# Thitrongdan202/Digital-Watermarking-for-image-Video-using-DCT-SVD-Singular-Value-Decomposition

Measured on AMD Instinct MI355X. Metric: frames/sec embed+extract @4K Y-channel, higher is better.
Workload: dtype f32

## Files before the change

### digital-watermarking-for-image-video-using-dct-svd-singular-value-decomposition_amd/csrc/wmhip.hip

```cpp
#include <hip/hip_runtime.h>
#include <stdio.h>
#include <stdlib.h>
#include <string.h>
#include <new>

#include "wm_internal.h"
#include "wm_tile_math.h"

using namespace wmi;

namespace wmi {

thread_local char g_err[512] = "";

int set_err(int code, const char* fmt, const char* a, const char* b) {
  snprintf(g_err, sizeof(g_err), fmt, a, b);
  return code;
}

int grow(wm_ctx* ctx, void** buf, size_t* have, size_t bytes, const char* what) {
  if (bytes <= *have) return WM_OK;
  if (*buf) {
    WM_HIP(hipStreamSynchronize(ctx->stream));
    WM_HIP(hipFree(*buf));
    *buf = nullptr; *have = 0;
  }
  const size_t mb = (size_t)1 << 20;
  const size_t want = (bytes + mb - 1) / mb * mb;
  if (hipMalloc(buf, want) != hipSuccess) {
    (void)hipGetLastError();
    *buf = nullptr;
    return set_err(WM_ERR_NOMEM, "hipMalloc failed for %s", what);
  }
  *have = want;
  return WM_OK;
}

}

namespace {

constexpr int N_SUMS = 5;

#if !defined(WM_NO_ASM_JACOBI)
#include "wm_jacobi_gfx950.inc"
#if !__has_include("wm_jacobi_sigma_gfx950.inc")
#error "wm_jacobi_sigma_gfx950.inc is generated: run `python tools/gen_jacobi_asm.py --write` (build() does) before compiling"
#endif
#include "wm_jacobi_sigma_gfx950.inc"
#endif

__device__ __forceinline__ int sigma_tile_dev(const wm::RawTile& raw, float (&s)[8]) {
#if !defined(WM_NO_ASM_JACOBI)
  float n2[8];
  constexpr float SIGMA_SKIP2 = 1e-8f;
  constexpr int SIGMA_SKIP_FROM = 2;
  const unsigned long long more = jacobi_sigma_gfx950(raw.lo, raw.hi, n2, wm::JAC_CONV2_SIGMA, SIGMA_SKIP2, 3, SIGMA_SKIP_FROM);
#pragma unroll
  for (int i = 0; i < 8; ++i) s[i] = wm::fsqrt(n2[i]);
  return more ? -1 : 1;
#else
  return wm::sigma_tile_pk(raw, s);
#endif
}

template <bool ALIGNED>
__device__ __forceinline__ uint32_t load_px4(const uint8_t* __restrict__ q) {
  if (ALIGNED) return *reinterpret_cast<const uint32_t*>(q);
  return q[0] | (q[1] << 8) | (q[2] << 16) | ((uint32_t)q[3] << 24);
}
template <bool ALIGNED>
__device__ __forceinline__ void store_px4(uint8_t* __restrict__ q, const uint32_t w) {
  if (ALIGNED) { *reinterpret_cast<uint32_t*>(q) = w; return; }
#pragma unroll
  for (int i = 0; i < 4; ++i) q[i] = (uint8_t)(w >> (8 * i));
}
template <bool ALIGNED>
__device__ __forceinline__ void load_px8(const uint8_t* __restrict__ q, uint32_t& lo, uint32_t& hi) {
  if (ALIGNED) { const uint2 w = *reinterpret_cast<const uint2*>(q); lo = w.x; hi = w.y; }
  else { lo = load_px4<false>(q); hi = load_px4<false>(q + 4); }
}
template <bool ALIGNED>
__device__ __forceinline__ void store_px8(uint8_t* __restrict__ q, const uint32_t lo, const uint32_t hi) {
  if (ALIGNED) *reinterpret_cast<uint2*>(q) = make_uint2(lo, hi);
  else { store_px4<false>(q, lo); store_px4<false>(q + 4, hi); }
}

template <bool ALIGNED>
__device__ __forceinline__ void load_raw(const uint8_t* __restrict__ p, const size_t stride, wm::RawTile& t) {
#pragma unroll
  for (int r = 0; r < 8; ++r) load_px8<ALIGNED>(p + r * stride, t.lo[r], t.hi[r]);
}

template <bool ALIGNED>
__device__ __forceinline__ void load_tile_u8(const uint8_t* __restrict__ p, const size_t stride, float (&a)[8][8]) {
#pragma unroll
  for (int r = 0; r < 8; ++r) {
    uint32_t lo, hi;
    load_px8<ALIGNED>(p + r * stride, lo, hi);
    a[r][0] = (float)(lo & 0xffu); a[r][1] = (float)((lo >> 8) & 0xffu);
    a[r][2] = (float)((lo >> 16) & 0xffu); a[r][3] = (float)(lo >> 24);
    a[r][4] = (float)(hi & 0xffu); a[r][5] = (float)((hi >> 8) & 0xffu);
    a[r][6] = (float)((hi >> 16) & 0xffu); a[r][7] = (float)(hi >> 24);
  }
}

template <bool ALIGNED>
__device__ __forceinline__ void store_tile_u8(uint8_t* __restrict__ p, const size_t stride, const float (&a)[8][8]) {
#pragma unroll
  for (int r = 0; r < 8; ++r) {
    const uint32_t lo = wm::quant_u8(a[r][0]) | (wm::quant_u8(a[r][1]) << 8) |
                        (wm::quant_u8(a[r][2]) << 16) | (wm::quant_u8(a[r][3]) << 24);
    const uint32_t hi = wm::quant_u8(a[r][4]) | (wm::quant_u8(a[r][5]) << 8) |
                        (wm::quant_u8(a[r][6]) << 16) | (wm::quant_u8(a[r][7]) << 24);
    store_px8<ALIGNED>(p + r * stride, lo, hi);
  }
}

template <bool ALIGNED>
__device__ __forceinline__ void load_words(const uint8_t* __restrict__ p, const size_t stride, uint32_t (&w)[8]) {
#pragma unroll
  for (int r = 0; r < 8; ++r) w[r] = load_px4<ALIGNED>(p + r * stride);
}
template <bool ALIGNED>
__device__ __forceinline__ void store_words(uint8_t* __restrict__ p, const size_t stride, const uint32_t (&w)[8]) {
#pragma unroll
  for (int r = 0; r < 8; ++r) store_px4<ALIGNED>(p + r * stride, w[r]);
}

template <bool VEC>
__device__ __forceinline__ void load_row8_f32(const float* __restrict__ p, float (&row)[8]) {
  if (VEC) {
    const float4 x = *reinterpret_cast<const float4*>(p);
    const float4 y = *reinterpret_cast<const float4*>(p + 4);
    row[0] = x.x; row[1] = x.y; row[2] = x.z; row[3] = x.w;
    row[4] = y.x; row[5] = y.y; row[6] = y.z; row[7] = y.w;
  } else {
#pragma unroll
    for (int i = 0; i < 8; ++i) row[i] = p[i];
  }
}

template <bool VEC>
__device__ __forceinline__ void store_row8_f32(float* __restrict__ p, const float (&row)[8]) {
  if (VEC) {
    *reinterpret_cast<float4*>(p) = make_float4(row[0], row[1], row[2], row[3]);
    *reinterpret_cast<float4*>(p + 4) = make_float4(row[4], row[5], row[6], row[7]);
  } else {
#pragma unroll
    for (int i = 0; i < 8; ++i) p[i] = row[i];
  }
}

__device__ __forceinline__ void load_mat_f32(const float* __restrict__ p, float (&m)[8][8]) {
#pragma unroll
  for (int r = 0; r < 8; ++r) load_row8_f32<true>(p + r * 8, m[r]);
}
__device__ __forceinline__ void store_mat_f32(float* __restrict__ p, const float (&m)[8][8]) {
#pragma unroll
  for (int r = 0; r < 8; ++r) store_row8_f32<true>(p + r * 8, m[r]);
}

struct Geom {
  int nbx;
  int n_tiles;
  int W;
  size_t HW;
  size_t row_stride;
  size_t plane_stride;
};

#define STRIDED_TILE(base, g, plane, ty, tx) \
  ((base) + (plane) * (g).plane_stride + (size_t)(ty) * 8 * (g).row_stride + (size_t)(tx) * 8)
#define DENSE_TILE(out, g, plane, ty, tx) ((out) + (plane) * (g).HW + (size_t)(ty) * 8 * (g).W + (size_t)(tx) * 8)

__device__ __forceinline__ bool tile_coords(const Geom& g, int& t, int& ty, int& tx) {
  t = blockIdx.x * WAVE + threadIdx.x;
  if (t >= g.n_tiles) return false;
  ty = t / g.nbx;
  tx = t - ty * g.nbx;
  return true;
}

constexpr unsigned N_XCD = 8;
struct GroupPlane { unsigned grp; size_t plane; };
__device__ __forceinline__ GroupPlane group_plane_planefast(const unsigned n_planes) {
  const unsigned b = blockIdx.x, x = b % N_XCD, k = b / N_XCD;
  return {x + N_XCD * (k / n_planes), k % n_planes};
}
__device__ __forceinline__ bool tile_coords_planefast(const Geom& g, const unsigned n_planes, int& t, int& ty,
                                                      int& tx, size_t& plane) {
  const GroupPlane gp = group_plane_planefast(n_planes);
  plane = gp.plane;
  t = (int)(gp.grp * WAVE + threadIdx.x);
  if (t >= g.n_tiles) return false;
  ty = t / g.nbx;
  tx = t - ty * g.nbx;
  return true;
}
inline dim3 tile_grid_planefast(const Geom& g, int n_planes) {
  const size_t groups = ((size_t)g.n_tiles + WAVE - 1) / WAVE;
  const size_t per_xcd = (groups + N_XCD - 1) / N_XCD;
  return dim3((unsigned)(per_xcd * N_XCD * (size_t)n_planes), 1, 1);
}

constexpr unsigned FB_SUB = 64;
constexpr unsigned FB_PAD = 32;
constexpr unsigned FB_KINDS = 4;
constexpr int EMBED_WAVES = 3;
constexpr int FALLBACK_WAVES = 2;

__device__ __forceinline__ size_t fb_counter(const unsigned l) { return (size_t)l * FB_PAD; }

template <typename Store>
__device__ __forceinline__ bool fb_reserve(int* __restrict__ fb_cnt, const unsigned kind, const unsigned sub, const bool flag,
                                           const Store& store) {
  const unsigned long long dmask = __builtin_amdgcn_ballot_w64(flag);
  if (dmask == 0ull) return flag;
  const unsigned lane = __builtin_amdgcn_mbcnt_hi(~0u, __builtin_amdgcn_mbcnt_lo(~0u, 0u));
  const unsigned leader = (unsigned)__builtin_ctzll(dmask);
  const unsigned l = kind * FB_SUB + sub;
  int base = 0;
  if (lane == leader) base = atomicAdd(fb_cnt + fb_counter(l), (int)__builtin_popcountll(dmask));
  base = __builtin_amdgcn_readlane(base, leader);
  return flag && store(l, base, (unsigned)__builtin_popcountll(dmask & ((1ull << lane) - 1ull)));
}

struct FlaggedTile {
  size_t plane;
  int t, ty, tx;
  size_t off;
  size_t slot;
};
struct FbWalk {
  const uint32_t* __restrict__ fb_list;
  uint32_t fb_cap, fb_cap3;
  int pre[FB_KINDS], total[FB_KINDS];

  __device__ __forceinline__ FbWalk(const uint32_t* __restrict__ fb_list_, const int* __restrict__ fb_cnt,
                                    const uint32_t fb_cap_, const uint32_t fb_cap3_)
      : fb_list(fb_list_), fb_cap(fb_cap_), fb_cap3(fb_cap3_) {
    static_assert(FB_SUB == WAVE, "one sub-list per lane");
#pragma unroll
    for (int k = 0; k < (int)FB_KINDS; ++k) {
      int c = fb_cnt[fb_counter(k * FB_SUB + threadIdx.x)];
      if (k == 3) c = min(c, (int)fb_cap3);
      int incl = c;
#pragma unroll
      for (int o = 1; o < WAVE; o <<= 1) { const int v = __shfl_up(incl, o, WAVE); if ((int)threadIdx.x >= o) incl += v; }
      pre[k] = incl - c;
      total[k] = __shfl(incl, WAVE - 1, WAVE);
    }
  }
  __device__ __forceinline__ bool item(const int k, const int it0, const Geom& g, FlaggedTile& tl) const {
    const int it = min(it0 + (int)threadIdx.x, total[k] - 1);
    int sub = 0;
#pragma unroll
    for (int o = WAVE / 2; o > 0; o >>= 1) { const int p = __shfl(pre[k], sub + o, WAVE); if (p <= it) sub += o; }
    const int j = it - __shfl(pre[k], sub, WAVE);
    if (it0 + (int)threadIdx.x >= total[k]) return false;
    tl.slot = (size_t)sub * (k == 3 ? fb_cap3 : fb_cap) + j;
    const uint32_t id = fb_list[(size_t)k * FB_SUB * fb_cap + tl.slot];
    tl.plane = id / (uint32_t)g.n_tiles;
    tl.t = (int)(id % (uint32_t)g.n_tiles);
    tl.ty = tl.t / g.nbx;
    tl.tx = tl.t - tl.ty * g.nbx;
    tl.off = STRIDED_TILE((size_t)0, g, tl.plane, tl.ty, tl.tx);
    return true;
  }
};

__device__ __forceinline__ void fill_alpha_k(const float alpha, const int K, float (&alpha_k)[8]) {
#pragma unroll
  for (int i = 0; i < 8; ++i) alpha_k[i] = (i < K) ? alpha : 0.0f;
}

template <bool ALIGNED, bool YW>
__device__ __forceinline__ void finish_flagged(const Geom& g, const FlaggedTile& tl, float* __restrict__ sigma_c, uint8_t* stego,
                                               float* __restrict__ yw, const float (&sc)[8], const float (&a)[8][8]) {
  store_row8_f32<true>(sigma_c + (tl.plane * g.n_tiles + tl.t) * 8, sc);
  store_tile_u8<ALIGNED>(stego + tl.off, g.row_stride, a);
  if (YW) {
    float* o = DENSE_TILE(yw, g, tl.plane, tl.ty, tl.tx);
#pragma unroll
    for (int r = 0; r < 8; ++r) store_row8_f32<false>(o + (size_t)r * g.W, a[r]);
  }
}

template <bool ALIGNED, bool YW>
__device__ __forceinline__ void embed_group(
    const uint8_t* host, const float* __restrict__ sigma_w,
    uint8_t* stego, float* __restrict__ sigma_c, float* __restrict__ yw,
    const Geom& g, const size_t sw_plane_stride, const float alpha, const int K,
    int* __restrict__ status, uint32_t* __restrict__ fb_list, int* __restrict__ fb_cnt, const uint32_t fb_cap,
    float* __restrict__ fb_b, const uint32_t fb_cap3,
    const int t, const int ty, const int tx, const size_t plane) {
  const size_t off = STRIDED_TILE((size_t)0, g, plane, ty, tx);
  const unsigned fb_sub = blockIdx.x % FB_SUB;
  auto append_kind = [&](const bool flag, const unsigned kind) {
    fb_reserve(fb_cnt, kind, fb_sub, flag, [&](const unsigned l, const int base, const unsigned rank) {
      fb_list[(size_t)l * fb_cap + base + rank] = (uint32_t)(plane * g.n_tiles + t);
      return true;
    });
  };
  wm::v2f a[4][8];
  float n2[8];
  int sweeps;
  bool cst;
  int r1;
  {
    wm::RawTile raw;
    load_raw<ALIGNED>(host + off, g.row_stride, raw);
    cst = false;
    if (__builtin_amdgcn_ballot_w64(raw.lo[0] == raw.hi[0] && raw.lo[0] == raw.hi[7]) != 0ull) cst = wm::raw_is_constant(raw);
    r1 = 0;
    if (__builtin_amdgcn_ballot_w64(!cst && wm::raw_rank1_pretest(raw)) != 0ull && !cst && wm::raw_is_rank1(raw)) r1 = 1;
    if (__builtin_amdgcn_ballot_w64(!cst && r1 == 0) == 0ull) {
      append_kind(cst, 1);
      append_kind(r1 != 0, 2);
      return;
    }
#if !defined(WM_NO_ASM_JACOBI)
    sweeps = jacobi_cols_gfx950(raw.lo, raw.hi, a, n2, wm::JAC_CONV2, wm::JAC_SKIP2, 4, 3) ? -1 : 1;
#else
    sweeps = wm::embed_jacobi_pk(raw, a, n2);
#endif
  }
  asm volatile("" ::: "memory");
  float e[8];
  bool deficient;
  {
    float sw[8], sc[8], alpha_k[8];
    load_row8_f32<true>(sigma_w + plane * sw_plane_stride + (size_t)t * 8, sw);
    fill_alpha_k(alpha, K, alpha_k);
    wm::embed_coeffs_pk(n2, sw, alpha_k, e, sc, deficient);
    deficient = deficient || cst || r1 != 0;
    if (!deficient) store_row8_f32<true>(sigma_c + (plane * g.n_tiles + t) * 8, sc);
  }
  bool one_small = deficient && !cst && r1 == 0;
  one_small = fb_reserve(fb_cnt, 3, fb_sub, one_small, [&](const unsigned, const int base, const unsigned rank) {
    const unsigned j = (unsigned)base + rank;
    if (j >= fb_cap3) return false;
    const size_t slot = (size_t)fb_sub * fb_cap3 + j;
    fb_list[(size_t)3 * FB_SUB * fb_cap + slot] = (uint32_t)(plane * g.n_tiles + t);
    wm::v2f* dstb = reinterpret_cast<wm::v2f*>(fb_b + slot * 64);
#pragma unroll
    for (int rp = 0; rp < 4; ++rp)
#pragma unroll
      for (int c = 0; c < 8; ++c) dstb[rp * 8 + c] = a[rp][c];
    return true;
  });
// ... 44 lines not shown
    if (!walk.item(0, it0, g, tl)) continue;
    load_tile_u8<ALIGNED>(host + tl.off, g.row_stride, a);
    load_row8_f32<true>(sigma_w + tl.plane * sw_plane_stride + (size_t)tl.t * 8, sw);
    if (wm::embed_tile_completed(a, sw, alpha_k, sc) < 0) atomicOr(status, 1);
    finish_flagged<ALIGNED, YW>(g, tl, sigma_c, stego, yw, sc, a);
  }
  for (int it0 = blockIdx.x * WAVE; it0 < walk.total[1]; it0 += gridDim.x * WAVE) {
    FlaggedTile tl;
    float a[8][8], sw[8], sc[8];
    if (!walk.item(1, it0, g, tl)) continue;
    const float v0 = (float)host[tl.off];
    load_row8_f32<true>(sigma_w + tl.plane * sw_plane_stride + (size_t)tl.t * 8, sw);
    const unsigned long long bm = __builtin_amdgcn_ballot_w64(v0 == 0.0f);
    if (bm == 0ull) wm::embed_tile_constant_t<1>(v0, sw, alpha_k, sc, a);
    else if (bm == __builtin_amdgcn_ballot_w64(true)) wm::embed_tile_constant_t<0>(v0, sw, alpha_k, sc, a);
    else wm::embed_tile_constant(v0, sw, alpha_k, sc, a);
    finish_flagged<ALIGNED, YW>(g, tl, sigma_c, stego, yw, sc, a);
  }
  for (int it0 = blockIdx.x * WAVE; it0 < walk.total[2]; it0 += gridDim.x * WAVE) {
    FlaggedTile tl;
    float a[8][8], sw[8], sc[8];
    if (!walk.item(2, it0, g, tl)) continue;
    load_tile_u8<ALIGNED>(host + tl.off, g.row_stride, a);
    load_row8_f32<true>(sigma_w + tl.plane * sw_plane_stride + (size_t)tl.t * 8, sw);
    wm::embed_tile_rank1(a, sw, alpha_k, sc, a);
    finish_flagged<ALIGNED, YW>(g, tl, sigma_c, stego, yw, sc, a);
  }
}

template <bool ALIGNED, bool YW>
__global__ __launch_bounds__(WAVE, 1) void k_embed_one_small(
    const uint8_t* host, const float* __restrict__ sigma_w,
    uint8_t* stego, float* __restrict__ sigma_c, float* __restrict__ yw,
    const Geom g, const size_t sw_plane_stride, const float alpha, const int K,
    int* __restrict__ status, const uint32_t* __restrict__ fb_list, const int* __restrict__ fb_cnt, const uint32_t fb_cap,
    const float* __restrict__ fb_b, const uint32_t fb_cap3) {
  float alpha_k[8];
  fill_alpha_k(alpha, K, alpha_k);
  const FbWalk walk(fb_list, fb_cnt, fb_cap, fb_cap3);
  for (int it0 = blockIdx.x * WAVE; it0 < walk.total[3]; it0 += gridDim.x * WAVE) {
    FlaggedTile tl;
    if (!walk.item(3, it0, g, tl)) continue;
    float a[8][8], bb[8][8], sw[8], sc[8];
    load_tile_u8<ALIGNED>(host + tl.off, g.row_stride, a);
    const wm::v2f* srcb = reinterpret_cast<const wm::v2f*>(fb_b + tl.slot * 64);
#pragma unroll
    for (int rp = 0; rp < 4; ++rp)
#pragma unroll
      for (int c = 0; c < 8; ++c) { const wm::v2f v = srcb[rp * 8 + c]; bb[2 * rp][c] = v[0]; bb[2 * rp + 1][c] = v[1]; }
    load_row8_f32<true>(sigma_w + tl.plane * sw_plane_stride + (size_t)tl.t * 8, sw);
    float n6 = 0.0f, n0 = 0.0f;
#pragma unroll
    for (int r = 0; r < 8; ++r) { n6 = __builtin_fmaf(bb[r][6], bb[r][6], n6); n0 = __builtin_fmaf(bb[r][0], bb[r][0], n0); }
    const bool one = n6 > wm::SIGMA_RATIO_MIN2 * n0;
    if (wm::wave_any(one)) { if (one) wm::embed_tile_one_small(a, bb, sw, alpha_k, sc, a); }
    if (wm::wave_any(!one)) { if (!one) wm::embed_tile_from_b(a, bb, sw, alpha_k, sc, a); }
    finish_flagged<ALIGNED, YW>(g, tl, sigma_c, stego, yw, sc, a);
  }
}

__global__ void k_copy_border(const uint8_t* host, uint8_t* stego,
                              float* __restrict__ yw, const int H, const int W, const int Hb,
                              const int Wb, const size_t row_stride, const size_t plane_stride) {
  const size_t plane = blockIdx.y;
  const int n_right = (W - Wb) * Hb;
  const int n_bottom = (H - Hb) * W;
  for (int i = blockIdx.x * blockDim.x + threadIdx.x; i < n_right + n_bottom;
       i += gridDim.x * blockDim.x) {
    int r, c;
    if (i < n_right) { r = i / (W - Wb); c = Wb + i % (W - Wb); }
    else { const int j = i - n_right; r = Hb + j / W; c = j % W; }
    const size_t o = plane * plane_stride + (size_t)r * row_stride + c;
    const uint8_t px = host[o];
    if (stego != host) stego[o] = px;
    if (yw) yw[plane * (size_t)H * W + (size_t)r * W + c] = (float)px;
  }
}

template <bool ALIGNED, typename Epi>
__global__ __launch_bounds__(WAVE, 3) void k_sigma_pass(const uint8_t* __restrict__ planes, const Geom g,
                                                    int* __restrict__ status, const Epi epi) {
  int t, ty, tx;
  if (!tile_coords(g, t, ty, tx)) return;
  const size_t plane = blockIdx.y;
  wm::RawTile raw;
  float s[8];
  load_raw<ALIGNED>(STRIDED_TILE(planes, g, plane, ty, tx), g.row_stride, raw);
  if (sigma_tile_dev(raw, s) < 0) atomicOr(status, 1);
  epi(raw, s, plane, t, plane * g.n_tiles + t);
}

struct EpiSigma {
  float* __restrict__ sigma;
  __device__ __forceinline__ void operator()(const wm::RawTile&, const float (&s)[8], size_t, int, const size_t ti) const {
    store_row8_f32<true>(sigma + ti * 8, s);
  }
};

struct EpiMask {
  const float* __restrict__ sigma_w;
  float* __restrict__ sw_eff;
  float* __restrict__ gain;
  uint8_t* __restrict__ black;
  size_t sw_plane_stride;
  float lo, hi;
  __device__ __forceinline__ void operator()(const wm::RawTile& raw, const float (&s)[8], const size_t plane, const int t,
                                             const size_t ti) const {
    float sw[8];
    const float gn = wm::mask_gain(s, lo, hi);
    if (sw_eff) {
      load_row8_f32<true>(sigma_w + plane * sw_plane_stride + (size_t)t * 8, sw);
      wm::mask_sigma_w(gn, sw);
      store_row8_f32<true>(sw_eff + ti * 8, sw);
    }
    if (gain) gain[ti] = gn;
    if (black) black[ti] = (wm::raw_is_constant(raw) && raw.lo[0] == 0u) ? 1 : 0;
  }
};

template <bool VECF>
__global__ __launch_bounds__(WAVE, 2) void k_svd_tiles(const float* __restrict__ planes,
                                                   float* __restrict__ U, float* __restrict__ S,
                                                   float* __restrict__ Vt, const Geom g,
                                                   int* __restrict__ status) {
  int t, ty, tx;
  if (!tile_coords(g, t, ty, tx)) return;
  const size_t plane = blockIdx.y;
  const float* p = STRIDED_TILE(planes, g, plane, ty, tx);
  float a[8][8], s[8], vt[8][8];
#pragma unroll
  for (int r = 0; r < 8; ++r) load_row8_f32<VECF>(p + (size_t)r * g.row_stride, a[r]);
  if (wm::svd_tile(a, s, vt) < 0) atomicOr(status, 1);
  const size_t ti = plane * g.n_tiles + t;
  const bool deficient = !(s[7] > 1e-5f * s[0]);
  if (!deficient) {
    store_row8_f32<true>(S + ti * 8, s);
    store_mat_f32(U + ti * 64, a);
    store_mat_f32(Vt + ti * 64, vt);
  }
  if (wm::wave_any(deficient)) {
    asm volatile("" ::: "memory");
#pragma unroll
    for (int r = 0; r < 8; ++r) load_row8_f32<VECF>(p + (size_t)r * g.row_stride, a[r]);
    if (wm::svd_tile(a, s, vt, true) < 0) atomicOr(status, 1);
    if (deficient) {
      store_row8_f32<true>(S + ti * 8, s);
      store_mat_f32(U + ti * 64, a);
      store_mat_f32(Vt + ti * 64, vt);
    }
  }
}

struct MaskParams { float lo, hi, cut; };
template <bool ALIGNED, bool VECF, bool PX, bool MM, bool MASK>
__global__ __launch_bounds__(WAVE, 3) void k_extract_tiles(
    const uint8_t* __restrict__ stego, const float* __restrict__ sigma_c,
    const float* __restrict__ Uw, const float* __restrict__ Vwt, float* __restrict__ out,
    const Geom g, const unsigned n_planes, const size_t uv_plane_stride, const float inv_alpha, const int K,
    int* __restrict__ status, unsigned* __restrict__ mm, const MaskParams mk) {
  int t, ty, tx;
  size_t plane;
  bool valid = true;
  if (MM) {
    const GroupPlane gp = group_plane_planefast(n_planes);
    plane = gp.plane;
    if ((size_t)gp.grp * WAVE >= (size_t)g.n_tiles) return;
    t = (int)(gp.grp * WAVE + threadIdx.x);
    valid = t < g.n_tiles;
    t = valid ? t : g.n_tiles - 1;
    ty = t / g.nbx; tx = t - ty * g.nbx;
  } else if (!tile_coords_planefast(g, n_planes, t, ty, tx, plane)) return;
  wm::RawTile raw;
  float a[8][8], s[8], sc[8], keep[8];
  load_raw<ALIGNED>(STRIDED_TILE(stego, g, plane, ty, tx), g.row_stride, raw);
  if (sigma_tile_dev(raw, s) < 0) atomicOr(status, 1);
  load_row8_f32<true>(sigma_c + (plane * g.n_tiles + t) * 8, sc);
  if (MASK) wm::mask_keep(sc, mk.lo, mk.hi, mk.cut, K, keep);
  else {
#pragma unroll
    for (int i = 0; i < 8; ++i) keep[i] = (i < K) ? 1.0f : 0.0f;
  }
  float uw[8][8], vwt[8][8];
  const size_t mi = (plane * uv_plane_stride + (size_t)t) * 64;
  load_mat_f32(Uw + mi, uw);
  load_mat_f32(Vwt + mi, vwt);
  if (PX) wm::extract_tile_px(s, sc, inv_alpha, keep, uw, vwt, a);
  else wm::extract_tile(s, sc, inv_alpha, keep, uw, vwt, a);
  float* o = DENSE_TILE(out, g, plane, ty, tx);
  if (valid) {
#pragma unroll
    for (int r = 0; r < 8; ++r) store_row8_f32<VECF>(o + (size_t)r * g.W, a[r]);
  }
  if (MM) {
    float lo = a[0][0], hi = a[0][0];
#pragma unroll
    for (int r = 0; r < 8; ++r)
#pragma unroll
      for (int c = 0; c < 8; ++c) { lo = fminf(lo, a[r][c]); hi = fmaxf(hi, a[r][c]); }
    unsigned ulo = f2ord(lo), uhi = f2ord(hi);
#pragma unroll
    for (int o_ = 32; o_ > 0; o_ >>= 1) { ulo = min(ulo, (unsigned)__shfl_down(ulo, o_, WAVE)); uhi = max(uhi, (unsigned)__shfl_down(uhi, o_, WAVE)); }
    if (threadIdx.x == 0) {
      const size_t groups = ((size_t)g.n_tiles + WAVE - 1) / WAVE, pair = plane * groups + group_plane_planefast(n_planes).grp;
      mm[2 * pair] = ulo; mm[2 * pair + 1] = uhi;
    }
  }
}

__global__ __launch_bounds__(256) void k_sum_planes(const float* __restrict__ in, const size_t plane_elems, const int n,
                                                   float* __restrict__ out) {
  for (size_t i = (size_t)blockIdx.x * blockDim.x + threadIdx.x; i < plane_elems; i += (size_t)gridDim.x * blockDim.x) {
    float acc = 0.0f;
    for (int z = 0; z < n; ++z) acc += in[(size_t)z * plane_elems + i];
    out[i] = acc;
  }
}

__global__ __launch_bounds__(WAVE) void k_factors_to_pixel(const float* Uw, const float* Vwt, float* Ux, float* Vxt,
                                                          const size_t n_tiles) {
  const size_t t = (size_t)blockIdx.x * WAVE + threadIdx.x;
  if (t >= n_tiles) return;
  float u[8][8], vt[8][8];
  load_mat_f32(Uw + t * 64, u);
  load_mat_f32(Vwt + t * 64, vt);
  wm::factors_to_pixel(u, vt);
  store_mat_f32(Ux + t * 64, u);
  store_mat_f32(Vxt + t * 64, vt);
}

template <bool VECF>
__global__ __launch_bounds__(WAVE, 3) void k_reconstruct_tiles(
    const float* __restrict__ Uw, const float* __restrict__ sw_hat,
    const float* __restrict__ Vwt, float* __restrict__ out, const Geom g) {
  int t, ty, tx;
  if (!tile_coords(g, t, ty, tx)) return;
  const size_t plane = blockIdx.y;
  const size_t ti = plane * g.n_tiles + t;
  float sh[8], zero[8], one[8], uw[8][8], vwt[8][8], a[8][8];
  load_row8_f32<true>(sw_hat + ti * 8, sh);
#pragma unroll
  for (int i = 0; i < 8; ++i) { zero[i] = 0.0f; one[i] = 1.0f; }
  load_mat_f32(Uw + ti * 64, uw);
  load_mat_f32(Vwt + ti * 64, vwt);
  wm::extract_tile(sh, zero, 1.0f, one, uw, vwt, a);
  float* o = DENSE_TILE(out, g, plane, ty, tx);
#pragma unroll
  for (int r = 0; r < 8; ++r) store_row8_f32<VECF>(o + (size_t)r * g.W, a[r]);
}

__device__ __forceinline__ double wave_sum(double x) {
#pragma unroll
  for (int o = 32; o > 0; o >>= 1) x += __shfl_down(x, o, WAVE);
  return x;
}

template <bool ALIGNED, bool MASK>
__global__ __launch_bounds__(WAVE, 3) void k_detect_tiles(
    const uint8_t* __restrict__ stego, const float* __restrict__ sigma_c,
    const float* __restrict__ sigma_w, double* __restrict__ partials, const Geom g,
    const size_t sw_plane_stride, const float inv_alpha, int* __restrict__ status, const MaskParams mk) {
  constexpr int NS = N_SUMS + (MASK ? 1 : 0);
  int t, ty, tx;
  const size_t plane = blockIdx.y;
  double acc[NS] = {};
  if (tile_coords(g, t, ty, tx)) {
    wm::RawTile raw;
    float s[8], sc[8], sw[8];
    load_raw<ALIGNED>(STRIDED_TILE(stego, g, plane, ty, tx), g.row_stride, raw);
    if (sigma_tile_dev(raw, s) < 0) atomicOr(status, 1);
    load_row8_f32<true>(sigma_c + (plane * g.n_tiles + t) * 8, sc);
    load_row8_f32<true>(sigma_w + plane * sw_plane_stride + (size_t)t * 8, sw);
    if (MASK) {
      float keep[8];
      const bool carried = wm::mask_keep(sc, mk.lo, mk.hi, mk.cut, 8, keep);
#pragma unroll
      for (int i = 0; i < 8; ++i) {
        if (i > 0 && !carried) continue;
        const double x = (double)sw[i];
        const double y = (double)((s[i] - sc[i]) * inv_alpha * keep[i]);
        acc[0] += x; acc[1] += y; acc[2] += x * y; acc[3] += x * x; acc[4] += y * y;
      }
      acc[N_SUMS] = carried ? 8.0 : 1.0;
    } else {
#pragma unroll
      for (int i = 0; i < 8; ++i) {
        const double x = (double)sw[i];
        const double y = (double)((s[i] - sc[i]) * inv_alpha);
        acc[0] += x; acc[1] += y; acc[2] += x * y; acc[3] += x * x; acc[4] += y * y;
      }
    }
  }
#pragma unroll
  for (int k = 0; k < NS; ++k) acc[k] = wave_sum(acc[k]);
  if (threadIdx.x == 0) {
    double* o = partials + (plane * gridDim.x + blockIdx.x) * NS;
#pragma unroll
    for (int k = 0; k < NS; ++k) o[k] = acc[k];
  }
}

template <bool MASK>
__global__ __launch_bounds__(256) void k_detect_finalize(const double* __restrict__ partials,
                                                        double* __restrict__ scores,
                                                        const int n_waves, double n_vals) {
  constexpr int NS = N_SUMS + (MASK ? 1 : 0);
  __shared__ double sm[4][NS];
  const size_t plane = blockIdx.x;
  double acc[NS] = {};
  for (int w = threadIdx.x; w < n_waves; w += blockDim.x) {
    const double* p = partials + (plane * n_waves + w) * NS;
#pragma unroll
    for (int k = 0; k < NS; ++k) acc[k] += p[k];
  }
#pragma unroll
  for (int k = 0; k < NS; ++k) acc[k] = wave_sum(acc[k]);
  if ((threadIdx.x & 63) == 0) {
#pragma unroll
    for (int k = 0; k < NS; ++k) sm[threadIdx.x >> 6][k] = acc[k];
  }
  __syncthreads();
  if (threadIdx.x == 0) {
    double s[NS];
#pragma unroll
    for (int k = 0; k < NS; ++k) s[k] = sm[0][k] + sm[1][k] + sm[2][k] + sm[3][k];
    if (MASK) n_vals = s[N_SUMS];
    double score = 0.0;
    if (n_vals > 0) {
      const double cov = s[2] - s[0] * s[1] / n_vals;
      double va = s[3] - s[0] * s[0] / n_vals;
      double vb = s[4] - s[1] * s[1] / n_vals;
      va = va > 0 ? va : 0;
      vb = vb > 0 ? vb : 0;
      score = cov / (sqrt(va) * sqrt(vb) + 1e-8);
    }
    scores[plane] = score;
  }
}

struct EpiPayloadSigmaW {
  const uint8_t* __restrict__ tile_bit;
  float* __restrict__ sw_eff;
  uint8_t* __restrict__ black;
  float delta;
  __device__ __forceinline__ void operator()(const wm::RawTile& raw, const float (&s)[8], size_t, const int t,
                                             const size_t ti) const {
    float sw[8];
    wm::payload_sigma_w(s, tile_bit[t] & 1, delta, sw);
    store_row8_f32<true>(sw_eff + ti * 8, sw);
    if (black) black[ti] = (wm::raw_is_constant(raw) && raw.lo[0] == 0u) ? 1 : 0;
  }
};

struct EpiPayloadSigmaWDither {
  const uint8_t* __restrict__ tile_bit;
  const uint16_t* __restrict__ tile_dither;
  float* __restrict__ sw_eff;
// ... 855 lines not shown
    return set_err(WM_ERR_BADARG, "votes / tile_bit_index is NULL or misaligned");
  const size_t lds = (size_t)n_bits * sizeof(int);
  if (lds > 48 * 1024)
    WM_HIP(hipFuncSetAttribute((const void*)k_payload_offset_scan, hipFuncAttributeMaxDynamicSharedMemorySize, (int)lds));
  hipLaunchKernelGGL(k_payload_offset_scan, dim3((unsigned)n_tx, (unsigned)n_ty), dim3(OFFSET_SCAN_THREADS), lds, ctx->stream, votes,
                     tile_bit_index, reinterpret_cast<long long*>(scores), ny, nx, nbx, n_bits);
  WM_HIP(hipGetLastError());
  return WM_OK;
}

int wm_payload_sigma1_scan_u8_dev(wm_ctx* ctx, const uint8_t* stego, float* s1, int n_planes, int h, int w, int row_stride,
                                  size_t plane_stride) {
  WM_TRY(check_plane_args(ctx, stego, n_planes, h, w, row_stride, plane_stride));
  const size_t pitch = (size_t)(h / 8) * (size_t)(w / 8);
  if (n_planes == 0 || pitch == 0) return WM_OK;
  if (pitch > (size_t)INT32_MAX) return set_err(WM_ERR_BADARG, "more than 2^31 - 1 tiles a plane");
  if (!s1 || ((uintptr_t)s1 & 3u)) return set_err(WM_ERR_BADARG, "s1 is NULL or misaligned");
  const PhaseGeom g{h, w, (int)pitch, (size_t)row_stride, plane_stride};
  const dim3 grid((unsigned)((pitch + WAVE - 1) / WAVE), 64, (unsigned)n_planes);
  hipLaunchKernelGGL(k_payload_phase_scan<EpiPhaseSigma1>, grid, dim3(WAVE), 0, ctx->stream, stego, g, ctx->d_status,
                     EpiPhaseSigma1{s1});
  WM_HIP(hipGetLastError());
  return WM_OK;
}

static int check_keyed_sizes(int h, int w, int nby, int nbx, float delta, size_t& spitch) {
  if (h < 8 || w < 8) return set_err(WM_ERR_BADARG, "a keyed search needs a whole tile (h, w >= 8)");
  if (nby < 0 || nbx < 0 || h / 8 > nby || w / 8 > nbx) return set_err(WM_ERR_BADARG, "the crop has more tiles than the table");
  WM_TRY(check_delta(delta));
  const size_t n_ty = (size_t)(nby - (h - 7) / 8) + 1, n_tx = (size_t)(nbx - (w - 7) / 8) + 1;
  if (nbx > 65535 || n_ty > 65535 || (size_t)nby * (size_t)nbx > (size_t)INT32_MAX || n_ty * n_tx > ((size_t)1 << 24))
    return set_err(WM_ERR_BADARG, "tile grid too large");
  spitch = n_ty * n_tx;
  return WM_OK;
}

int wm_payload_keyed_scores_dev(wm_ctx* ctx, const float* s1, const uint16_t* tile_dither, int64_t* scores, int h, int w, int nby,
                                int nbx, float delta) {
  WM_TRY(wmi::use_ctx(ctx));
  size_t spitch;
  WM_TRY(check_keyed_sizes(h, w, nby, nbx, delta, spitch));
  if (!tile_dither || ((uintptr_t)tile_dither & 1u)) return set_err(WM_ERR_BADARG, "tile_dither is NULL or at an odd address");
  if (!s1 || !scores || ((uintptr_t)s1 & 3u) || ((uintptr_t)scores & 7u)) return set_err(WM_ERR_BADARG, "s1 / scores is NULL or misaligned");
  WM_HIP(hipMemsetAsync(scores, 0, 64 * spitch * sizeof(int64_t), ctx->stream));
  const KeyedGeom g{h, w, nby, nbx, (h / 8) * (w / 8), spitch};
  const long long n_tx = nbx - w / 8 + 1, nx = w / 8, n_tx_max = nbx - (w - 7) / 8 + 1;
  const bool windows = nx * ((n_tx + WAVE - 1) / WAVE) >= 2 * n_tx * ((nx + WAVE - 1) / WAVE);
  const dim3 grid((unsigned)(windows ? n_tx_max : (n_tx_max + WAVE - 1) / WAVE), (unsigned)(nby - (h - 7) / 8 + 1), 64);
  hipLaunchKernelGGL(windows ? k_payload_keyed_scan_windows : k_payload_keyed_scan, grid, dim3(WAVE), 0, ctx->stream, s1, tile_dither,
                     reinterpret_cast<long long*>(scores), g, delta, 1.0f / (2.0f * delta));
  WM_HIP(hipGetLastError());
  return WM_OK;
}

static int check_keyed_best_sizes(int n_anchor, int n_tables, int n_cand, int h, int w, int nby, int nbx, float delta) {
  size_t spitch;
  WM_TRY(check_keyed_sizes(h, w, nby, nbx, delta, spitch));
  if (n_anchor < 1 || n_cand < 1 || n_tables < 1) return set_err(WM_ERR_BADARG, "n_anchor, n_tables and n_cand must be at least 1");
  if ((size_t)(h / 8) * (size_t)(w / 8) * (size_t)n_anchor >= ((size_t)1 << 24))
    return set_err(WM_ERR_BADARG, "(h / 8) (w / 8) n_anchor must stay below 2^24 (a score below 2^39)");
  return WM_OK;
}

int wm_payload_keyed_best_dev(wm_ctx* ctx, const float* s1, int n_anchor, const uint16_t* tables, int n_tables, const int32_t* table_of,
                              int n_cand, int64_t* best, int h, int w, int nby, int nbx, float delta) {
  WM_TRY(wmi::use_ctx(ctx));
  WM_TRY(check_keyed_best_sizes(n_anchor, n_tables, n_cand, h, w, nby, nbx, delta));
  if (!tables || ((uintptr_t)tables & 1u)) return set_err(WM_ERR_BADARG, "tables is NULL or at an odd address");
  if (!s1 || !table_of || !best || (((uintptr_t)s1 | (uintptr_t)table_of) & 3u) || ((uintptr_t)best & 7u))
    return set_err(WM_ERR_BADARG, "s1 / table_of / best is NULL or misaligned");
  long long* const b = reinterpret_cast<long long*>(best);
  WM_HIP(hipMemsetAsync(best, 0xFF, (size_t)n_cand * 64 * 2 * sizeof(int64_t), ctx->stream));
  const KeyedGeom g{h, w, nby, nbx, (h / 8) * (w / 8), 0};
  const long long n_tx = nbx - w / 8 + 1, nx = w / 8, n_tx_max = nbx - (w - 7) / 8 + 1;
  const bool windows = nx * ((n_tx + WAVE - 1) / WAVE) >= 2 * n_tx * ((nx + WAVE - 1) / WAVE);
  constexpr int CHUNK = 1023;
  for (int c0 = 0; c0 < n_cand; c0 += CHUNK) {
    const int nc = std::min(CHUNK, n_cand - c0);
    const KeyedBestArgs a{s1, tables, table_of + (size_t)c0 * n_anchor, b + (size_t)c0 * 128, n_anchor, n_tables};
    const dim3 grid((unsigned)(windows ? n_tx_max : (n_tx_max + WAVE - 1) / WAVE), (unsigned)(nby - (h - 7) / 8 + 1), (unsigned)(64 * nc));
    hipLaunchKernelGGL(windows ? k_payload_keyed_best_windows : k_payload_keyed_best, grid, dim3(WAVE), 0, ctx->stream, a, g, delta,
                       1.0f / (2.0f * delta));
    WM_HIP(hipGetLastError());
  }
  const size_t n = (size_t)n_cand * 64;
  hipLaunchKernelGGL(k_payload_keyed_best_unpack, dim3((unsigned)((n + 255) / 256)), dim3(256), 0, ctx->stream, b, n);
  WM_HIP(hipGetLastError());
  return WM_OK;
}

static int check_k7_sizes(const int32_t* llr, int n_info, int n_codewords, size_t llr_stride, const uint8_t* info_bits) {
  if (n_info < 1) return set_err(WM_ERR_BADARG, "n_info must be at least 1");
  if (n_info > wm::K7_MAX_STEPS - wm::K7_TAIL) return set_err(WM_ERR_BADARG, "n_info + 6 steps exceed 2^18");
  if (n_codewords < 1) return set_err(WM_ERR_BADARG, "n_codewords must be at least 1");
  if (llr_stride < 2 * (size_t)(n_info + wm::K7_TAIL)) return set_err(WM_ERR_BADARG, "llr_stride < 2 (n_info + 6)");
  if (!llr || !info_bits) return set_err(WM_ERR_BADARG, "llr / info_bits is NULL");
  return WM_OK;
}

int wm_payload_decode_k7_dev(wm_ctx* ctx, const int32_t* llr, int n_info, int n_codewords, size_t llr_stride, uint8_t* info_bits,
                             int32_t* final_metric, uint64_t* decisions) {
  WM_TRY(wmi::use_ctx(ctx));
  WM_TRY(check_k7_sizes(llr, n_info, n_codewords, llr_stride, info_bits));
  if (((uintptr_t)llr | (uintptr_t)final_metric) & 3u || ((uintptr_t)decisions & 7u))
    return set_err(WM_ERR_BADARG, "llr / final_metric / decisions is misaligned");
  if (!decisions) {
    WM_TRY(wmi::grow(ctx, &ctx->sigma_ws, &ctx->sigma_ws_bytes,
                     (size_t)n_codewords * (size_t)(n_info + wm::K7_TAIL) * sizeof(uint64_t), "decision words"));
    decisions = static_cast<uint64_t*>(ctx->sigma_ws);
  }
  hipLaunchKernelGGL(k_payload_viterbi, dim3((unsigned)n_codewords), dim3(WAVE), 0, ctx->stream, llr, n_info, llr_stride, info_bits,
                     final_metric, reinterpret_cast<unsigned long long*>(decisions));
  WM_HIP(hipGetLastError());
  return WM_OK;
}

int wm_svd_tiles_f32_dev(wm_ctx* ctx, const float* planes, float* U, float* S, float* Vt,
                         int n_planes, int H, int W, int row_stride, size_t plane_stride) {
  WM_TRY(check_plane_args(ctx, planes, n_planes, H, W, row_stride, plane_stride));
  const Geom g = make_geom(H, W, row_stride, plane_stride);
  if (n_planes == 0 || g.n_tiles == 0) return WM_OK;
  if (!U || !S || !Vt || (((uintptr_t)U | (uintptr_t)S | (uintptr_t)Vt) & 15u))
    return set_err(WM_ERR_BADARG, "U/S/Vt is NULL or not 16-byte aligned");
  const dim3 grid = tile_grid(g, n_planes), block(WAVE);
  with_bools([&](auto V) {
    hipLaunchKernelGGL((k_svd_tiles<V.value>), grid, block, 0, ctx->stream, planes, U, S, Vt, g, ctx->d_status);
  }, f32_vec_ok(planes, (size_t)row_stride, plane_stride));
  WM_HIP(hipGetLastError());
  return WM_OK;
}

static int extract_tiles_dev(wm_ctx* ctx, const uint8_t* stego, const float* sigma_c, const float* Uw,
                             const float* Vwt, float* out, int n_planes, int H, int W, int row_stride,
                             size_t plane_stride, size_t uv_plane_stride, float alpha, int K, bool px, unsigned* mm = nullptr,
                             const MaskParams* mask = nullptr) {
  WM_TRY(check_plane_args(ctx, stego, n_planes, H, W, row_stride, plane_stride));
  if (mask) WM_TRY(check_mask(mask->lo, mask->hi, mask->cut));
  if (!out) return set_err(WM_ERR_BADARG, "out is NULL");
  if (K < 0 || K > 8) return set_err(WM_ERR_BADARG, "K must be in 0..8");
  if (n_planes == 0 || H == 0 || W == 0) return WM_OK;
  const Geom g = make_geom(H, W, row_stride, plane_stride);
  if ((H % 8) || (W % 8))
    WM_HIP(hipMemsetAsync(out, 0, (size_t)n_planes * g.HW * sizeof(float), ctx->stream));
  if (g.n_tiles == 0) return WM_OK;
  if (!sigma_c || !Uw || !Vwt || (((uintptr_t)sigma_c | (uintptr_t)Uw | (uintptr_t)Vwt) & 15u))
    return set_err(WM_ERR_BADARG, "sigma_c/Uw/Vwt is NULL or not 16-byte aligned");
  if (uv_plane_stride != 0 && uv_plane_stride != (size_t)g.n_tiles)
    return set_err(WM_ERR_BADARG, "uv_plane_stride must be 0 (shared) or n_tiles");
  const float inv_alpha = 1.0f / fmaxf(alpha, 1e-8f);
  const bool al = u8_aligned(stego, stego, row_stride, plane_stride);
  const bool vf = f32_vec_ok(out, (size_t)W, g.HW);
  if ((((size_t)g.n_tiles + WAVE - 1) / WAVE + N_XCD) * (size_t)n_planes > 0x7fffffffull)
    return set_err(WM_ERR_BADARG, "more than 2^31 tile groups in one call");
  const dim3 grid = tile_grid_planefast(g, n_planes), block(WAVE);
  const MaskParams mk = mask ? *mask : MaskParams{0.0f, 1.0f, 1.0f};
  with_bools([&](auto P, auto A, auto V, auto M, auto T) {
    hipLaunchKernelGGL((k_extract_tiles<A.value, V.value, P.value, M.value, T.value>), grid, block, 0, ctx->stream, stego, sigma_c,
                       Uw, Vwt, out, g, (unsigned)n_planes, uv_plane_stride, inv_alpha, K, ctx->d_status, mm, mk);
  }, px, al, vf, mm != nullptr, mask != nullptr);
  WM_HIP(hipGetLastError());
  return WM_OK;
}

int wm_extract_tiles_u8_dev(wm_ctx* ctx, const uint8_t* stego, const float* sigma_c, const float* Uw,
                            const float* Vwt, float* out, int n_planes, int H, int W, int row_stride,
                            size_t plane_stride, size_t uv_plane_stride, float alpha, int K) {
  return extract_tiles_dev(ctx, stego, sigma_c, Uw, Vwt, out, n_planes, H, W, row_stride, plane_stride,
                           uv_plane_stride, alpha, K, false);
}

int wm_extract_tiles_px_u8_dev(wm_ctx* ctx, const uint8_t* stego, const float* sigma_c, const float* Ux,
                               const float* Vxt, float* out, int n_planes, int H, int W, int row_stride,
                               size_t plane_stride, size_t uv_plane_stride, float alpha, int K) {
  return extract_tiles_dev(ctx, stego, sigma_c, Ux, Vxt, out, n_planes, H, W, row_stride, plane_stride,
                           uv_plane_stride, alpha, K, true);
}

int wm_extract_tiles_masked_u8_dev(wm_ctx* ctx, const uint8_t* stego, const float* sigma_c, const float* Uw,
                                   const float* Vwt, float* out, int n_planes, int H, int W, int row_stride,
                                   size_t plane_stride, size_t uv_plane_stride, float alpha, int K, float lo, float hi, float cut) {
  const MaskParams mk{lo, hi, cut};
  return extract_tiles_dev(ctx, stego, sigma_c, Uw, Vwt, out, n_planes, H, W, row_stride, plane_stride,
                           uv_plane_stride, alpha, K, false, nullptr, &mk);
}

int wm_extract_tiles_px_masked_u8_dev(wm_ctx* ctx, const uint8_t* stego, const float* sigma_c, const float* Ux,
                                      const float* Vxt, float* out, int n_planes, int H, int W, int row_stride,
                                      size_t plane_stride, size_t uv_plane_stride, float alpha, int K, float lo, float hi, float cut) {
  const MaskParams mk{lo, hi, cut};
  return extract_tiles_dev(ctx, stego, sigma_c, Ux, Vxt, out, n_planes, H, W, row_stride, plane_stride,
                           uv_plane_stride, alpha, K, true, nullptr, &mk);
}

static int extract_unscrambled_dev(wm_ctx* ctx, const uint8_t* stego, const float* sigma_c, const float* Uw, const float* Vwt,
                                   const wm_route* route, uint8_t* out, int n_planes, int H, int W, int row_stride,
                                   size_t plane_stride, size_t uv_plane_stride, float alpha, int K, int px, int do_norm,
                                   const MaskParams* mask) {
  WM_TRY(check_plane_args(ctx, stego, n_planes, H, W, row_stride, plane_stride));
  if (!out || !route) return set_err(WM_ERR_BADARG, "out / route is NULL");
  if (n_planes == 0 || H == 0 || W == 0) return WM_OK;
  const size_t n = (size_t)H * W;
  const Geom g = make_geom(H, W, row_stride, plane_stride);
  const size_t groups = ((size_t)g.n_tiles + WAVE - 1) / WAVE;
  float* w; unsigned* mm;
  WM_TRY(staged(ctx, &ctx->extract_f32, &ctx->extract_f32_bytes, "extract staging", [&](Carve& cv) {
    w = cv.take<float>((size_t)n_planes * n);
    mm = cv.take<unsigned>((size_t)n_planes * groups * 2);
  }));
  const bool use_mm = do_norm && g.n_tiles > 0;
  WM_TRY(extract_tiles_dev(ctx, stego, sigma_c, Uw, Vwt, w, n_planes, H, W, row_stride, plane_stride, uv_plane_stride, alpha, K,
                           px != 0, use_mm ? mm : nullptr, mask));
  return wmi::route_unpermute_normalize(ctx, w, route, out, n, n_planes, do_norm, use_mm ? mm : nullptr, (unsigned)groups,
                                        ((H % 8) || (W % 8)) ? 1 : 0);
}

int wm_extract_unscrambled_u8_dev(wm_ctx* ctx, const uint8_t* stego, const float* sigma_c, const float* Uw, const float* Vwt,
                                  const wm_route* route, uint8_t* out, int n_planes, int H, int W, int row_stride,
                                  size_t plane_stride, size_t uv_plane_stride, float alpha, int K, int px, int do_norm) {
  return extract_unscrambled_dev(ctx, stego, sigma_c, Uw, Vwt, route, out, n_planes, H, W, row_stride, plane_stride,
                                 uv_plane_stride, alpha, K, px, do_norm, nullptr);
}

int wm_extract_unscrambled_masked_u8_dev(wm_ctx* ctx, const uint8_t* stego, const float* sigma_c, const float* Uw,
                                         const float* Vwt, const wm_route* route, uint8_t* out, int n_planes, int H, int W,
                                         int row_stride, size_t plane_stride, size_t uv_plane_stride, float alpha, int K, int px,
                                         int do_norm, float lo, float hi, float cut) {
  const MaskParams mk{lo, hi, cut};
  return extract_unscrambled_dev(ctx, stego, sigma_c, Uw, Vwt, route, out, n_planes, H, W, row_stride, plane_stride,
                                 uv_plane_stride, alpha, K, px, do_norm, &mk);
}

int wm_tile_factors_to_pixel_dev(wm_ctx* ctx, const float* Uw, const float* Vwt, float* Ux, float* Vxt,
                                 size_t n_tiles) {
  WM_TRY(wmi::use_ctx(ctx));
  if (n_tiles == 0) return WM_OK;
  if (!Uw || !Vwt || !Ux || !Vxt || (((uintptr_t)Uw | (uintptr_t)Vwt | (uintptr_t)Ux | (uintptr_t)Vxt) & 15u))
    return set_err(WM_ERR_BADARG, "factor arrays are NULL or not 16-byte aligned");
  if (n_tiles > ((size_t)1 << 31)) return set_err(WM_ERR_BADARG, "too many tiles");
  hipLaunchKernelGGL(k_factors_to_pixel, dim3((unsigned)((n_tiles + WAVE - 1) / WAVE)), dim3(WAVE), 0, ctx->stream,
                     Uw, Vwt, Ux, Vxt, n_tiles);
  WM_HIP(hipGetLastError());
  return WM_OK;
}

int wm_reconstruct_tiles_dev(wm_ctx* ctx, const float* Uw, const float* sw_hat, const float* Vwt,
                             float* out, int n_planes, int H, int W) {
  WM_TRY(wmi::use_ctx(ctx));
  if (n_planes < 0 || H < 0 || W < 0 || n_planes > 65535) return set_err(WM_ERR_BADARG, "bad size");
  if (!out) return set_err(WM_ERR_BADARG, "out is NULL");
  if (n_planes == 0 || H == 0 || W == 0) return WM_OK;
  const Geom g = make_geom(H, W, W, (size_t)H * W);
  if ((H % 8) || (W % 8))
    WM_HIP(hipMemsetAsync(out, 0, (size_t)n_planes * g.HW * sizeof(float), ctx->stream));
  if (g.n_tiles == 0) return WM_OK;
  if (!Uw || !sw_hat || !Vwt || (((uintptr_t)Uw | (uintptr_t)sw_hat | (uintptr_t)Vwt) & 15u))
    return set_err(WM_ERR_BADARG, "Uw/sw_hat/Vwt is NULL or not 16-byte aligned");
  const dim3 grid = tile_grid(g, n_planes), block(WAVE);
  with_bools([&](auto V) {
    hipLaunchKernelGGL((k_reconstruct_tiles<V.value>), grid, block, 0, ctx->stream, Uw, sw_hat, Vwt, out, g);
  }, f32_vec_ok(out, (size_t)W, g.HW));
  WM_HIP(hipGetLastError());
  return WM_OK;
}

static int detect_tiles_dev(wm_ctx* ctx, const uint8_t* stego, const float* sigma_c,
                            const float* sigma_w, double* scores, int n_planes, int H, int W,
                            int row_stride, size_t plane_stride, size_t sigma_w_plane_stride,
                            float alpha, const MaskParams* mask) {
  WM_TRY(check_plane_args(ctx, stego, n_planes, H, W, row_stride, plane_stride));
  if (mask) WM_TRY(check_mask(mask->lo, mask->hi, mask->cut));
  const int ns = N_SUMS + (mask ? 1 : 0);
  const MaskParams mk = mask ? *mask : MaskParams{0.0f, 1.0f, 1.0f};
  if (!scores) return set_err(WM_ERR_BADARG, "scores is NULL");
  if (n_planes == 0) return WM_OK;
  const Geom g = make_geom(H, W, row_stride, plane_stride);
  const int n_waves = (g.n_tiles + WAVE - 1) / WAVE;
  if (g.n_tiles > 0) {
    if (!sigma_c || !sigma_w || (((uintptr_t)sigma_c | (uintptr_t)sigma_w) & 15u) ||
        (sigma_w_plane_stride & 3u))
      return set_err(WM_ERR_BADARG, "sigma_c/sigma_w is NULL or not 16-byte aligned");
    WM_TRY(grow(ctx, &ctx->partials, &ctx->partials_bytes,
                (size_t)n_planes * n_waves * ns * sizeof(double), "detect partial sums"));
    const float inv_alpha = 1.0f / fmaxf(alpha, 1e-8f);
    const dim3 grid = tile_grid(g, n_planes), block(WAVE);
    with_bools([&](auto A, auto T) {
      hipLaunchKernelGGL((k_detect_tiles<A.value, T.value>), grid, block, 0, ctx->stream, stego, sigma_c, sigma_w,
                         (double*)ctx->partials, g, sigma_w_plane_stride, inv_alpha, ctx->d_status, mk);
    }, u8_aligned(stego, stego, row_stride, plane_stride), mask != nullptr);
    WM_HIP(hipGetLastError());
  }
  with_bools([&](auto T) {
    hipLaunchKernelGGL((k_detect_finalize<T.value>), dim3((unsigned)n_planes), dim3(256), 0, ctx->stream,
                       (const double*)ctx->partials, scores, n_waves, (double)g.n_tiles * 8.0);
  }, mask != nullptr && g.n_tiles > 0);
  WM_HIP(hipGetLastError());
  return WM_OK;
}

int wm_detect_tiles_u8_dev(wm_ctx* ctx, const uint8_t* stego, const float* sigma_c,
                           const float* sigma_w, double* scores, int n_planes, int H, int W,
                           int row_stride, size_t plane_stride, size_t sigma_w_plane_stride,
                           float alpha) {
  return detect_tiles_dev(ctx, stego, sigma_c, sigma_w, scores, n_planes, H, W, row_stride, plane_stride,
                          sigma_w_plane_stride, alpha, nullptr);
}

int wm_detect_tiles_masked_u8_dev(wm_ctx* ctx, const uint8_t* stego, const float* sigma_c, const float* sigma_w,
                                  double* scores, int n_planes, int H, int W, int row_stride, size_t plane_stride,
                                  size_t sigma_w_plane_stride, float alpha, float lo, float hi, float cut) {
  const MaskParams mk{lo, hi, cut};
  return detect_tiles_dev(ctx, stego, sigma_c, sigma_w, scores, n_planes, H, W, row_stride, plane_stride,
                          sigma_w_plane_stride, alpha, &mk);
// ... 433 lines not shown
```

Before: 23770.

## Share watermark U/Vt factors across planes via LDS staging in extract kernel

When the watermark factors are shared across planes (uv_plane_stride 0, at least two planes), the extract kernel now runs four waves per block, one per plane. The block cooperatively loads the Uw/Vwt tiles for its tile group into padded LDS once, and each wave reads them from there. This cuts repeated global loads of the 8x8 factor matrices per plane, in exchange for an LDS allocation, a block barrier, and idle waves when the plane count is not a multiple of four. The benchmark is a single Y channel, so this path probably does not run unless several frames are batched as planes.

```diff
diff --git a/digital-watermarking-for-image-video-using-dct-svd-singular-value-decomposition_amd/csrc/wmhip.hip b/digital-watermarking-for-image-video-using-dct-svd-singular-value-decomposition_amd/csrc/wmhip.hip
--- a/digital-watermarking-for-image-video-using-dct-svd-singular-value-decomposition_amd/csrc/wmhip.hip
+++ b/digital-watermarking-for-image-video-using-dct-svd-singular-value-decomposition_amd/csrc/wmhip.hip
@@ -161,6 +161,36 @@
   for (int r = 0; r < 8; ++r) store_row8_f32<true>(p + r * 8, m[r]);
 }
 
+constexpr int SH_WAVES = 4;
+constexpr int STAGE_PITCH4 = 17;
+constexpr int STAGE_MAT4 = WAVE * STAGE_PITCH4;
+constexpr int STAGE_LOADS = 2 * WAVE * 16 / (SH_WAVES * WAVE);
+typedef float stage4 __attribute__((ext_vector_type(4)));
+__device__ __forceinline__ void stage_fetch(const float* __restrict__ ublk, const float* __restrict__ vblk, const int last,
+                                            const int tid, stage4 (&raw)[STAGE_LOADS]) {
+#pragma unroll
+  for (int i = 0; i < STAGE_LOADS; ++i) {
+    const int q = i * (SH_WAVES * WAVE) + tid, r = q & (WAVE * 16 - 1);
+    const float* blk = (q < WAVE * 16) ? ublk : vblk;
+    raw[i] = *reinterpret_cast<const stage4*>(blk + (size_t)min(r >> 4, last) * 64 + (r & 15) * 4);
+  }
+}
+__device__ __forceinline__ void stage_put(stage4* __restrict__ lds, const int tid, const stage4 (&raw)[STAGE_LOADS]) {
+#pragma unroll
+  for (int i = 0; i < STAGE_LOADS; ++i) {
+    const int q = i * (SH_WAVES * WAVE) + tid, r = q & (WAVE * 16 - 1);
+    lds[(q < WAVE * 16 ? 0 : STAGE_MAT4) + (r >> 4) * STAGE_PITCH4 + (r & 15)] = raw[i];
+  }
+}
+__device__ __forceinline__ void stage_read(const stage4* __restrict__ blk, const int lane, float (&m)[8][8]) {
+#pragma unroll
+  for (int k = 0; k < 16; ++k) {
+    const stage4 v = blk[lane * STAGE_PITCH4 + k];
+    m[k / 2][(k & 1) * 4 + 0] = v.x; m[k / 2][(k & 1) * 4 + 1] = v.y;
+    m[k / 2][(k & 1) * 4 + 2] = v.z; m[k / 2][(k & 1) * 4 + 3] = v.w;
+  }
+}
+
 struct Geom {
   int nbx;
   int n_tiles;
@@ -187,16 +217,6 @@
 __device__ __forceinline__ GroupPlane group_plane_planefast(const unsigned n_planes) {
   const unsigned b = blockIdx.x, x = b % N_XCD, k = b / N_XCD;
   return {x + N_XCD * (k / n_planes), k % n_planes};
-}
-__device__ __forceinline__ bool tile_coords_planefast(const Geom& g, const unsigned n_planes, int& t, int& ty,
-                                                      int& tx, size_t& plane) {
-  const GroupPlane gp = group_plane_planefast(n_planes);
-  plane = gp.plane;
-  t = (int)(gp.grp * WAVE + threadIdx.x);
-  if (t >= g.n_tiles) return false;
-  ty = t / g.nbx;
-  tx = t - ty * g.nbx;
-  return true;
 }
 inline dim3 tile_grid_planefast(const Geom& g, int n_planes) {
   const size_t groups = ((size_t)g.n_tiles + WAVE - 1) / WAVE;
@@ -547,24 +567,32 @@
 }
 
 struct MaskParams { float lo, hi, cut; };
-template <bool ALIGNED, bool VECF, bool PX, bool MM, bool MASK>
-__global__ __launch_bounds__(WAVE, 3) void k_extract_tiles(
+template <bool ALIGNED, bool VECF, bool PX, bool MM, bool MASK, bool SH>
+__global__ __launch_bounds__(SH ? SH_WAVES * WAVE : WAVE, 3) void k_extract_tiles(
     const uint8_t* __restrict__ stego, const float* __restrict__ sigma_c,
     const float* __restrict__ Uw, const float* __restrict__ Vwt, float* __restrict__ out,
     const Geom g, const unsigned n_planes, const size_t uv_plane_stride, const float inv_alpha, const int K,
     int* __restrict__ status, unsigned* __restrict__ mm, const MaskParams mk) {
-  int t, ty, tx;
-  size_t plane;
+  __shared__ stage4 stage[SH ? 2 * STAGE_MAT4 : 1];
+  const int lane = threadIdx.x & (WAVE - 1);
+  const GroupPlane gp = group_plane_planefast(SH ? (n_planes + SH_WAVES - 1) / SH_WAVES : n_planes);
+  const size_t plane = SH ? gp.plane * SH_WAVES + __builtin_amdgcn_readfirstlane(threadIdx.x / WAVE) : gp.plane;
+  if ((size_t)gp.grp * WAVE >= (size_t)g.n_tiles) return;
+  if (SH) {
+    stage4 fetched[STAGE_LOADS];
+    stage_fetch(Uw + (size_t)gp.grp * WAVE * 64, Vwt + (size_t)gp.grp * WAVE * 64,
+                min((int)WAVE, g.n_tiles - (int)(gp.grp * WAVE)) - 1, threadIdx.x, fetched);
+    stage_put(stage, threadIdx.x, fetched);
+    __syncthreads();
+    if (plane >= n_planes) return;
+  }
+  int t = (int)(gp.grp * WAVE) + lane;
   bool valid = true;
   if (MM) {
-    const GroupPlane gp = group_plane_planefast(n_planes);
-    plane = gp.plane;
-    if ((size_t)gp.grp * WAVE >= (size_t)g.n_tiles) return;
-    t = (int)(gp.grp * WAVE + threadIdx.x);
     valid = t < g.n_tiles;
     t = valid ? t : g.n_tiles - 1;
-    ty = t / g.nbx; tx = t - ty * g.nbx;
-  } else if (!tile_coords_planefast(g, n_planes, t, ty, tx, plane)) return;
+  } else if (t >= g.n_tiles) return;
+  const int ty = t / g.nbx, tx = t - ty * g.nbx;
   wm::RawTile raw;
   float a[8][8], s[8], sc[8], keep[8];
   load_raw<ALIGNED>(STRIDED_TILE(stego, g, plane, ty, tx), g.row_stride, raw);
@@ -576,9 +604,14 @@
     for (int i = 0; i < 8; ++i) keep[i] = (i < K) ? 1.0f : 0.0f;
   }
   float uw[8][8], vwt[8][8];
-  const size_t mi = (plane * uv_plane_stride + (size_t)t) * 64;
-  load_mat_f32(Uw + mi, uw);
-  load_mat_f32(Vwt + mi, vwt);
+  if (SH) {
+    stage_read(stage, lane, uw);
+    stage_read(stage + STAGE_MAT4, lane, vwt);
+  } else {
+    const size_t mi = (plane * uv_plane_stride + (size_t)t) * 64;
+    load_mat_f32(Uw + mi, uw);
+    load_mat_f32(Vwt + mi, vwt);
+  }
   if (PX) wm::extract_tile_px(s, sc, inv_alpha, keep, uw, vwt, a);
   else wm::extract_tile(s, sc, inv_alpha, keep, uw, vwt, a);
   float* o = DENSE_TILE(out, g, plane, ty, tx);
@@ -595,8 +628,8 @@
     unsigned ulo = f2ord(lo), uhi = f2ord(hi);
 #pragma unroll
     for (int o_ = 32; o_ > 0; o_ >>= 1) { ulo = min(ulo, (unsigned)__shfl_down(ulo, o_, WAVE)); uhi = max(uhi, (unsigned)__shfl_down(uhi, o_, WAVE)); }
-    if (threadIdx.x == 0) {
-      const size_t groups = ((size_t)g.n_tiles + WAVE - 1) / WAVE, pair = plane * groups + group_plane_planefast(n_planes).grp;
+    if (lane == 0) {
+      const size_t groups = ((size_t)g.n_tiles + WAVE - 1) / WAVE, pair = plane * groups + gp.grp;
       mm[2 * pair] = ulo; mm[2 * pair + 1] = uhi;
     }
   }
@@ -1758,12 +1791,13 @@
   const bool vf = f32_vec_ok(out, (size_t)W, g.HW);
   if ((((size_t)g.n_tiles + WAVE - 1) / WAVE + N_XCD) * (size_t)n_planes > 0x7fffffffull)
     return set_err(WM_ERR_BADARG, "more than 2^31 tile groups in one call");
-  const dim3 grid = tile_grid_planefast(g, n_planes), block(WAVE);
+  const bool sh = uv_plane_stride == 0 && n_planes >= 2;
+  const dim3 grid = tile_grid_planefast(g, sh ? (n_planes + SH_WAVES - 1) / SH_WAVES : n_planes), block(sh ? SH_WAVES * WAVE : WAVE);
   const MaskParams mk = mask ? *mask : MaskParams{0.0f, 1.0f, 1.0f};
-  with_bools([&](auto P, auto A, auto V, auto M, auto T) {
-    hipLaunchKernelGGL((k_extract_tiles<A.value, V.value, P.value, M.value, T.value>), grid, block, 0, ctx->stream, stego, sigma_c,
-                       Uw, Vwt, out, g, (unsigned)n_planes, uv_plane_stride, inv_alpha, K, ctx->d_status, mm, mk);
-  }, px, al, vf, mm != nullptr, mask != nullptr);
+  with_bools([&](auto P, auto A, auto V, auto M, auto T, auto S) {
+    hipLaunchKernelGGL((k_extract_tiles<A.value, V.value, P.value, M.value, T.value, S.value>), grid, block, 0, ctx->stream, stego,
+                       sigma_c, Uw, Vwt, out, g, (unsigned)n_planes, uv_plane_stride, inv_alpha, K, ctx->d_status, mm, mk);
+  }, px, al, vf, mm != nullptr, mask != nullptr, sh);
   WM_HIP(hipGetLastError());
   return WM_OK;
 }
```

Measured after the change: 24070 (median of 6 runs). 1.3% higher.
